# abignoli/EdgeGraph3D

Hardware: AMD Instinct MI355X
Metric: triangulated edge-points/sec (higher is better)
Workload: dtype f64

## Files before the change

edgegraph3d_amd/api.py:

```python
import ctypes as C
import os

import numpy as np

from . import _cdefs as D

_LIB = None


class Eg3dError(RuntimeError):
    pass


def lib_path():
    return os.environ.get("EG3D_LIB") or os.path.join(os.path.dirname(os.path.abspath(__file__)), "libeg3d.so")


def lib():
    global _LIB
    if _LIB is None:
        path = lib_path()
        if not os.path.exists(path):
            raise Eg3dError("libeg3d.so (HIP extension) is missing: run `python -m edgegraph3d_amd.build`. "
                            "There is no CPU fallback.")
        L = C.CDLL(path)
        L.eg3d_last_error.restype = C.c_char_p
        L.eg3d_device_count.restype = C.c_int
        L.eg3d_dlt_rows.restype = C.c_int
        L.eg3d_create.argtypes = [C.POINTER(D.Scene), C.c_int, C.POINTER(C.c_void_p)]
        L.eg3d_destroy.argtypes = [C.c_void_p]
        L.eg3d_clone.argtypes = [C.c_void_p, C.POINTER(C.c_void_p)]
        L.eg3d_get_grid.argtypes = [C.c_void_p, C.c_int, C.c_int, D.u32p, D.u32p, C.POINTER(D.u32p), C.POINTER(D.u32p)]
        L.eg3d_candidates_run.argtypes = [C.c_void_p, C.POINTER(D.Seeds), C.c_uint32, C.c_uint32, C.POINTER(D.Candidates)]
        L.eg3d_free_candidates.argtypes = [C.POINTER(D.Candidates)]
        L.eg3d_match_refpoints.argtypes = [C.c_void_p, C.POINTER(D.Seeds), C.c_uint32, C.c_uint32, C.c_int,
                                           C.POINTER(D.EdgePoints), C.POINTER(D.StageTimes)]
        L.eg3d_free_edgepoints.argtypes = [C.POINTER(D.EdgePoints)]
        L.eg3d_upload_seeds.argtypes = [C.c_void_p, C.POINTER(D.Seeds)]
        L.eg3d_match_resident.argtypes = [C.c_void_p, C.c_uint32, C.c_uint32, C.c_int, C.POINTER(D.EdgePoints),
                                          C.POINTER(D.StageTimes)]
        L.eg3d_match_polyline_sets.argtypes = [C.c_void_p, C.POINTER(D.PolylineSets), C.c_uint32, C.c_uint32, C.c_int,
                                               C.POINTER(D.EdgePoints), C.POINTER(D.StageTimes)]
        L.eg3d_check_polyline_sets.argtypes = [C.POINTER(D.PolylineSets), C.c_int32]
        L.eg3d_last_device_output.argtypes = [C.c_void_p, C.POINTER(D.DeviceEdgePoints)]
        L.eg3d_set_pipelining.argtypes = [C.c_void_p, C.c_int, C.c_int]
        L.eg3d_gn_filter.argtypes = [C.c_void_p, D.f32p, D.u32p, D.i32p, D.f32p, C.c_uint64, C.c_float, C.c_int,
                                     D.f32p, D.u8p, D.f32p]
        _LIB = L
    return _LIB


EXPORTED_SYMBOLS = [
    "eg3d_last_error", "eg3d_device_count", "eg3d_dlt_rows", "eg3d_create", "eg3d_clone", "eg3d_destroy", "eg3d_get_grid", "eg3d_candidates_run",
    "eg3d_free_candidates", "eg3d_match_refpoints", "eg3d_free_edgepoints", "eg3d_upload_seeds",
    "eg3d_match_resident", "eg3d_gn_filter", "eg3d_last_device_output", "eg3d_match_polyline_sets", "eg3d_check_polyline_sets", "eg3d_set_pipelining",
]


def _check(rc, what):
    if rc != 0:
        raise Eg3dError("%s failed (rc=%d): %s" % (what, rc, lib().eg3d_last_error().decode()))


def check_polyline_sets(n_sets, row_off, pl_ids, n_views):
    row_off = np.ascontiguousarray(row_off, np.uint32)
    pl_ids = np.ascontiguousarray(pl_ids if len(pl_ids) else [0], np.uint32)
    ps = D.PolylineSets(n_sets, D.np_ptr(row_off, C.c_uint32), D.np_ptr(pl_ids, C.c_uint32))
    _check(lib().eg3d_check_polyline_sets(C.byref(ps), n_views), "eg3d_check_polyline_sets")


def device_count():
    return int(lib().eg3d_device_count())


class Context:
    def __init__(self, scene_ptr, device=0, _handle=None):
        self._h = C.c_void_p()
        if _handle is not None:
            self._h = _handle
        else:
            _check(lib().eg3d_create(scene_ptr, device, C.byref(self._h)), "eg3d_create")

    def clone(self):
        h = C.c_void_p()
        _check(lib().eg3d_clone(self._h, C.byref(h)), "eg3d_clone")
        return Context(None, _handle=h)

    def set_pipelining(self, lanes=0, units=0):
        _check(lib().eg3d_set_pipelining(self._h, lanes, units), "eg3d_set_pipelining")

    def close(self):
        if self._h:
            lib().eg3d_destroy(self._h)
            self._h = C.c_void_p()

    def __del__(self):
        try:
            self.close()
        except Exception:
            pass

    def grid(self, view, which):
        ncols, nrows = C.c_uint32(), C.c_uint32()
        off, ids = D.u32p(), D.u32p()
        _check(lib().eg3d_get_grid(self._h, view, which, C.byref(ncols), C.byref(nrows), C.byref(off), C.byref(ids)),
               "eg3d_get_grid")
        n = ncols.value * nrows.value
        o = D.as_np(off, n + 1, np.uint32)
        return ncols.value, nrows.value, o, D.as_np(ids, int(o[-1]), np.uint32)

    def upload_seeds(self, seeds_ptr):
        _check(lib().eg3d_upload_seeds(self._h, seeds_ptr), "eg3d_upload_seeds")

    def match_resident(self, begin, end, device_only=False):
        e, tm = D.EdgePoints(), D.StageTimes()
        rc = lib().eg3d_match_resident(self._h, begin, end, 1 if device_only else 0, C.byref(e), C.byref(tm))
        _check(rc, "eg3d_match_resident")
        if device_only:
            d = {"n_points": int(e.n_points), "n_obs": int(e.n_obs), "n_tasks": int(e.n_tasks),
                 "n_hypotheses": int(e.n_hypotheses), "n_chains": int(e.n_chains), "flags": int(e.flags)}
        else:
            d = D.edgepoints_to_dict(e)
        lib().eg3d_free_edgepoints(C.byref(e))
        d["times"] = {f[0]: getattr(tm, f[0]) for f in D.StageTimes._fields_}
        return d

    def time_match_to_host(self, begin, end):
        import time
        e, tm = D.EdgePoints(), D.StageTimes()
        t0 = time.perf_counter()
        rc = lib().eg3d_match_resident(self._h, begin, end, 0, C.byref(e), C.byref(tm))
        dt = time.perf_counter() - t0
        _check(rc, "eg3d_match_resident")
        n = int(e.n_points)
        lib().eg3d_free_edgepoints(C.byref(e))
        return dt, n

    def time_match_sets_to_host(self, n_sets, row_off, pl_ids):
        import time
        row_off = np.ascontiguousarray(row_off, np.uint32)
        pl_ids = np.ascontiguousarray(pl_ids if len(pl_ids) else [0], np.uint32)
        ps = D.PolylineSets(n_sets, D.np_ptr(row_off, C.c_uint32), D.np_ptr(pl_ids, C.c_uint32))
# ... 109 lines not shown
```

edgegraph3d_amd/csrc/eg3d_api.hip:

```cpp
#include <hip/hip_runtime.h>
#include <hipcub/hipcub.hpp>

#include <algorithm>
#include <cstdio>
#include <cstdlib>
#include <sys/mman.h>

#include <atomic>
#include <chrono>
#include <cmath>
#include <condition_variable>
#include <cstring>
#include <memory>
#include <mutex>
#include <shared_mutex>
#include <string>
#include <thread>
#include <vector>

#include "../../include/eg3d.h"
#include "../../include/eg3d_host.h"
#include "eg3d_host_copy.h"
#include "eg3d_kernels.h"

// ... 25 lines not shown
      g_err = std::string("hipMalloc(") + std::to_string(want) + "): " + hipGetErrorString(e);
      return EG3D_ERR_HIP;
    }
    cap = want;
    return EG3D_OK;
  }
  int ensure_keep(size_t bytes, size_t keep, hipStream_t st) {
    if (bytes <= cap && p) return EG3D_OK;
    if (!p || !keep) return ensure(bytes);
    void* q = nullptr;
    const size_t want = bytes + bytes / 2;
    hipError_t e = hipMalloc(&q, want);
    if (e != hipSuccess) {
      g_err = std::string("hipMalloc(") + std::to_string(want) + "): " + hipGetErrorString(e);
      return EG3D_ERR_HIP;
    }
    e = hipMemcpyAsync(q, p, keep, hipMemcpyDeviceToDevice, st);
    if (e == hipSuccess) e = hipStreamSynchronize(st);
    if (e != hipSuccess) {
      (void)hipFree(q);
      g_err = std::string("growing a device buffer: ") + hipGetErrorString(e);
      return EG3D_ERR_HIP;
    }
    (void)hipFree(p);
    p = q;
    cap = want;
    return EG3D_OK;
  }
  void release() {
    if (p) (void)hipFree(p);
    p = nullptr;
    cap = 0;
  }
  template <typename T>
  T* as() const {
    return reinterpret_cast<T*>(p);
  }
};

#define BUF_TRY(expr)          \
  do {                         \
    int _r = (expr);           \
    if (_r != EG3D_OK) return _r; \
  } while (0)

struct DevOwner {
  int device = 0;
  std::vector<void*> ptrs;
  ~DevOwner() {
    (void)hipSetDevice(device);
    for (void* p : ptrs)
      if (p) (void)hipFree(p);
  }
};
struct HostGrids {
  std::mutex mu;
  bool have[2] = {false, false};
  std::vector<std::vector<uint32_t>> h_off[2], h_ids[2];
  int device = 0, n_views = 0;
  const uint32_t* d_off[2] = {nullptr, nullptr};
  const uint32_t* d_ids[2] = {nullptr, nullptr};
  uint32_t cells_per_view[2] = {0, 0};
};

#ifndef EG3D_K3B_ENGINE_DEFAULT
#define EG3D_K3B_ENGINE_DEFAULT 0
#endif
struct Tunables {
  bool grid_on_host = false;
  int lanes = 0, units = 0, test_fail_unit = 0;
  int copy_threads = 0;
  double unit_ramp = 0.6;
  int lane_priorities = 1;
  static constexpr int kHostCallLanes = 3;
  int k3a_engine_waves = 0, k3a_engine_lanes = 0;
  int k3b_engine = EG3D_K3B_ENGINE_DEFAULT, k3c_waves = 0, k3c_lanes = 0;
  bool assume_short = false;
  bool trace_arena = false;
  bool k3b_full = false;
  uint32_t arena_cap0 = 0, hyp_cap = 0;
  uint32_t chain_cap0 = 0, pool_cap0 = 0;
  size_t max_scratch = 0;
  uint32_t slots_per_xcd = 0;
  bool use_lpt = true;
  static Tunables from_env() {
    Tunables t;
    if (const char* e = getenv("EG3D_K3A_ENGINE_WAVES")) t.k3a_engine_waves = atoi(e);
    if (const char* e = getenv("EG3D_K3A_ENGINE_LANES")) t.k3a_engine_lanes = atoi(e);
    if (const char* e = getenv("EG3D_K3B_ENGINE")) t.k3b_engine = atoi(e);
    if (const char* e = getenv("EG3D_K3C_WAVES")) t.k3c_waves = atoi(e);
    if (const char* e = getenv("EG3D_K3C_LANES")) t.k3c_lanes = atoi(e);
    if (const char* e = getenv("EG3D_K3B_ASSUME_SHORT")) t.assume_short = e[0] == '1';
    if (const char* e = getenv("EG3D_HYP_CAP")) t.hyp_cap = (uint32_t)std::max(1, atoi(e));
    if (const char* e = getenv("EG3D_ARENA_CAP0")) t.arena_cap0 = (uint32_t)std::max(16, atoi(e));
    if (const char* e = getenv("EG3D_CHAIN_CAP0")) t.chain_cap0 = (uint32_t)std::max(8, atoi(e));
    if (const char* e = getenv("EG3D_POOL_CAP0")) t.pool_cap0 = (uint32_t)std::max(64, atoi(e));
    if (const char* e = getenv("EG3D_MAX_SCRATCH_MB")) t.max_scratch = (size_t)std::max(1, atoi(e)) << 20;
    if (const char* e = getenv("EG3D_NO_LPT")) t.use_lpt = !(e[0] == '1');
    if (const char* e = getenv("EG3D_TRACE_ARENA")) t.trace_arena = e[0] == '1';
    if (const char* e = getenv("EG3D_K3B_FULL")) t.k3b_full = e[0] == '1';
    if (const char* e = getenv("EG3D_SLOTS_PER_XCD")) t.slots_per_xcd = (uint32_t)std::max(1, atoi(e));
    if (const char* e = getenv("EG3D_PIPELINE_LANES")) t.lanes = std::min(16, std::max(0, atoi(e)));
    if (const char* e = getenv("EG3D_TEST_FAIL_UNIT")) t.test_fail_unit = atoi(e);
    if (const char* e = getenv("EG3D_GRID_ON_HOST")) t.grid_on_host = e[0] == '1';
    if (const char* e = getenv("EG3D_COPY_THREADS_PER_LANE")) t.copy_threads = std::min(32, std::max(1, atoi(e)));
    if (const char* e = getenv("EG3D_LANE_PRIORITIES")) t.lane_priorities = atoi(e);
    if (const char* e = getenv("EG3D_UNIT_RAMP")) t.unit_ramp = std::min(16.0, std::max(1.0 / 16.0, atof(e)));
    if (const char* e = getenv("EG3D_PIPELINE_UNITS")) t.units = std::min(4096, std::max(0, atoi(e)));
    return t;
  }
};

struct eg3d_ctx {
  int device = 0;
  Tunables tune;
  hipStream_t stream = nullptr;
  int V = 0, W = 0, H = 0;
  DevScene ds;
  DevBuf b_camP, b_F, b_Fv, b_vpo, b_pvo, b_vtx, b_pls, b_ple, b_g30o, b_g30i, b_g4o, b_g4i, b_bbo, b_bb;
  std::shared_ptr<DevOwner> scene_owner;
  std::shared_ptr<HostGrids> hg;
  uint32_t gw[2] = {0, 0}, gh[2] = {0, 0};
  uint32_t grid_dropped = 0;
  uint32_t n_seeds = 0;
  std::shared_ptr<std::vector<uint32_t>> h_trk;
  DevBuf b_toff, b_tview, b_txy;
  std::shared_ptr<DevOwner> seeds_owner;
  DevBuf b_sv_seed, b_map_view, b_map_entry, b_map_n, b_raw_cnt, b_raw_off, b_cand_pl, b_start_hits, b_cand_cnt,
      b_start_cnt, b_task_off, b_task_seed, b_task_entry, b_task_hit, b_task_k, b_task_list_off, b_list_cnt, b_list_ptr,
      b_hits, b_tasks, b_nhyp, b_hyp_off, b_res, b_arena, b_ctr, b_cs_task, b_valid, b_chain_off, b_chains,
      b_cscratch, b_couts, b_cpts, b_cobs, b_cpoff, b_cooff, b_scan_tmp, b_scanchk, b_cost, b_cidx, b_cost2, b_order, b_redo[2];
  DevBuf o_X, o_off, o_view, o_pl, o_seg, o_xy, o_key;
  DevBuf f_X, f_off, f_view, f_xy, f_Xo, f_inl;
  DevBuf b_sets_off, b_sets_ids;
  DevBuf b_fscratch, b_queue, b_items;
  DevBuf b_pools, b_stage_pts, b_stage_obs, b_stage_used;
  uint32_t slots_per_xcd = 0;
  int k3c_per_cu = 0;
  bool k3b_long_latched = false;
  uint32_t max_pl_vtx = 0;
  uint64_t stage_cap_pts = 0, stage_cap_obs = 0;
  hipEvent_t ea[8], eb[8];
  hipEvent_t ecopy[7] = {nullptr, nullptr, nullptr, nullptr, nullptr, nullptr, nullptr};
  uint32_t chain_cap = 384, pool_cap = 0, hyp_cap = 160;
  uint32_t n_simd = 0;
  int wall_clock_khz = 0;
  double arena_per_hyp = 16.0;
  void* pinned = nullptr;
  size_t pinned_cap = 0, ring_chunk = 0;
  uint32_t* mbox = nullptr;
  uint32_t* mbox_dev = nullptr;
  uint32_t mbox_seq = 0;
  uint64_t last_np = 0, last_no = 0;
  int last_chunks = 0;
  bool last_accumulated = false;
  uint32_t last_nc = 0;
  uint32_t last_nhyp = 0;
  std::vector<eg3d_ctx*> lanes;
  bool is_lane = false;
  uint32_t host_calls = 0;
  uint64_t last_host_cloud_bytes = 0;
};

#ifndef EG3D_D2H_CHUNK
#define EG3D_D2H_CHUNK ((size_t)16 << 20)
#endif
#define EG3D_D2H_CHUNK_SMALL ((size_t)2 << 20)
#define EG3D_D2H_BIG_CLOUD ((size_t)96 << 20)
#ifndef EG3D_D2H_RING
#define EG3D_D2H_RING 4
#endif
static int ensure_d2h_ring(eg3d_ctx* c, size_t cloud_bytes) {
  const size_t want = cloud_bytes >= EG3D_D2H_BIG_CLOUD ? EG3D_D2H_CHUNK : EG3D_D2H_CHUNK_SMALL;
  if (c->pinned && c->ring_chunk >= want) return EG3D_OK;
  if (c->pinned) (void)hipHostFree(c->pinned);
  c->pinned = nullptr;
  c->ring_chunk = c->pinned_cap = 0;
  HIP_TRY(hipHostMalloc(&c->pinned, want * EG3D_D2H_RING, hipHostMallocDefault));
  c->ring_chunk = want;
  c->pinned_cap = want * EG3D_D2H_RING;
  return EG3D_OK;
}

template <typename T>
static int upload(DevBuf& b, const T* src, size_t n, hipStream_t st) {
  BUF_TRY(b.ensure(sizeof(T) * std::max<size_t>(n, 1)));
  if (n) HIP_TRY(hipMemcpyAsync(b.p, src, sizeof(T) * n, hipMemcpyHostToDevice, st));
  return EG3D_OK;
}

static int scan_exclusive_u32(eg3d_ctx* c, const uint32_t* in, uint32_t* out, size_t n_plus_one) {
  size_t tmp_bytes = 0;
  HIP_TRY(hipcub::DeviceScan::ExclusiveSum(nullptr, tmp_bytes, in, out, (int)n_plus_one, c->stream));
  BUF_TRY(c->b_scan_tmp.ensure(tmp_bytes));
  HIP_TRY(hipcub::DeviceScan::ExclusiveSum(c->b_scan_tmp.p, tmp_bytes, in, out, (int)n_plus_one, c->stream));
  return EG3D_OK;
}
static int ensure_mailbox(eg3d_ctx* c) {
  if (!c->mbox) {
    void* h = nullptr;
    HIP_TRY(hipHostMalloc(&h, sizeof(uint32_t) * EG3D_MBOX_WORDS, hipHostMallocMapped | hipHostMallocCoherent));
    memset(h, 0, sizeof(uint32_t) * EG3D_MBOX_WORDS);
    void* d = nullptr;
    if (hipHostGetDevicePointer(&d, h, 0) != hipSuccess) {
      (void)hipHostFree(h);
      g_err = "eg3d: hipHostGetDevicePointer failed for the read-back mailbox";
      return EG3D_ERR_HIP;
    }
    c->mbox = (uint32_t*)h;
    c->mbox_dev = (uint32_t*)d;
  }
  if (!c->b_scanchk.p) {
    BUF_TRY(c->b_scanchk.ensure(8 * sizeof(uint32_t)));
    HIP_TRY(hipMemsetAsync(c->b_scanchk.p, 0, 8 * sizeof(uint32_t), c->stream));
  }
// ... 405 lines not shown
        rc = EG3D_ERR_HIP;
      }
      if (rc != EG3D_OK) ok = false;
    }
    if (!ok) {
      if (rc == EG3D_OK) {
        g_err = "eg3d_create: grid construction failed";
        rc = EG3D_ERR_ARG;
      }
      eg3d_destroy(c);
      return rc;
    }
  }
  d.g30_w = (int)c->gw[0];
  d.g30_h = (int)c->gh[0];
  d.g4_w = (int)c->gw[1];
  d.g4_h = (int)c->gh[1];
  d.g30_off = c->b_g30o.as<uint32_t>();
  d.g30_ids = c->b_g30i.as<uint32_t>();
  d.g4_off = c->b_g4o.as<uint32_t>();
  d.g4_ids = c->b_g4i.as<uint32_t>();
  {
    bool mid = true;
    for (size_t v = 0; v < (size_t)V && mid; v++)
      for (int k = 0; k < 12 && mid; k++) {
        const float p = sc->cam_P[v * 16 + k];
        if (p != 0.0f) {
          const float a = p < 0 ? -p : p;
          mid = a >= 7.888609052210118e-31f && a <= 1.2676506002282294e+30f;
        }
      }
    d.cams_mid_range = mid ? 1 : 0;
  }
  c->max_pl_vtx = 0;
  for (uint32_t p = 0; p < NP; p++)
    if (sc->pl_valid[p]) c->max_pl_vtx = std::max(c->max_pl_vtx, sc->pl_vtx_off[p + 1] - sc->pl_vtx_off[p]);
  c->pool_cap = std::min<uint32_t>(131072, 768u * (uint32_t)std::min(V, 128));
  if (c->pool_cap < 6144) c->pool_cap = 6144;
  if (c->tune.pool_cap0) c->pool_cap = c->tune.pool_cap0;
  if (c->tune.chain_cap0) c->chain_cap = c->tune.chain_cap0;
  hipDeviceProp_t prop;
  HIP_TRY(hipGetDeviceProperties(&prop, device));
  c->n_simd = (uint32_t)prop.multiProcessorCount * 4;
  if (hipDeviceGetAttribute(&c->wall_clock_khz, hipDeviceAttributeWallClockRate, device) != hipSuccess) c->wall_clock_khz = 0;
  {
    const int per_cu = k3b_blocks_per_cu();
    if (per_cu < 1) {
      g_err = "eg3d_create: occupancy query of the expand kernel failed";
      eg3d_destroy(c);
      return EG3D_ERR_HIP;
    }
    const uint32_t cus = (uint32_t)prop.multiProcessorCount;
    const uint32_t n_xcd = std::min(8u, std::max(1u, cus / 32u));
    const uint32_t cus_per_xcd = std::max<uint32_t>((cus + n_xcd - 1u) / n_xcd, 40u);
    c->slots_per_xcd = ((uint32_t)per_cu + 1u) * cus_per_xcd + 16u;
    if (c->tune.slots_per_xcd) c->slots_per_xcd = c->tune.slots_per_xcd;
    if (c->tune.k3b_engine != 0) {
#ifdef EG3D_WITH_K3C_ENGINE
      c->k3c_per_cu = k3c_blocks_per_cu();
      if (c->k3c_per_cu < 1) {
        g_err = "eg3d_create: occupancy query of the expand engine failed";
        eg3d_destroy(c);
        return EG3D_ERR_HIP;
      }
#else
      g_err = "eg3d_create: EG3D_K3B_ENGINE=1, but this library was built without the lane-per-chain engine "
              "(-DEG3D_WITH_K3C_ENGINE: edgegraph3d_amd/variants/libeg3d_engine.so)";
      eg3d_destroy(c);
      return EG3D_ERR_ARG;
#endif
    }
  }
  HIP_TRY(hipStreamSynchronize(c->stream));
  c->scene_owner = std::make_shared<DevOwner>();
  c->scene_owner->device = device;
  for (DevBuf* b : scene_bufs(c)) c->scene_owner->ptrs.push_back(b->p);
  *out = c;
  return EG3D_OK;
}

extern "C" int eg3d_clone(eg3d_ctx* parent, eg3d_ctx** out) {
  if (!parent || !out) {
    g_err = "eg3d_clone: bad arguments";
    return EG3D_ERR_ARG;
  }
  HIP_TRY(hipSetDevice(parent->device));
  eg3d_ctx* c = new eg3d_ctx();
  c->device = parent->device;
  c->tune = parent->tune;
  HIP_TRY(hipStreamCreateWithFlags(&c->stream, hipStreamNonBlocking));
  for (int i = 0; i < 8; i++) {
    HIP_TRY(hipEventCreate(&c->ea[i]));
    HIP_TRY(hipEventCreate(&c->eb[i]));
  }
  for (int i = 0; i < 7; i++) HIP_TRY(hipEventCreateWithFlags(&c->ecopy[i], hipEventDisableTiming));
  c->V = parent->V;
  c->W = parent->W;
  c->H = parent->H;
  c->ds = parent->ds;
  {
    std::vector<DevBuf*> src = scene_bufs(parent), dst = scene_bufs(c);
    for (size_t i = 0; i < src.size(); i++) *dst[i] = *src[i];
  }
  c->scene_owner = parent->scene_owner;
  c->hg = parent->hg;
  for (int k = 0; k < 2; k++) {
    c->gw[k] = parent->gw[k];
    c->gh[k] = parent->gh[k];
  }
  c->grid_dropped = parent->grid_dropped;
  c->n_seeds = parent->n_seeds;
  c->h_trk = parent->h_trk;
  c->b_toff = parent->b_toff;
  c->b_tview = parent->b_tview;
  c->b_txy = parent->b_txy;
  c->seeds_owner = parent->seeds_owner;
  c->chain_cap = parent->chain_cap;
  c->pool_cap = parent->pool_cap;
  c->hyp_cap = parent->hyp_cap;
  c->n_simd = parent->n_simd;
  c->wall_clock_khz = parent->wall_clock_khz;
  c->arena_per_hyp = parent->arena_per_hyp;
  c->slots_per_xcd = parent->slots_per_xcd;
  c->k3c_per_cu = parent->k3c_per_cu;
  c->k3b_long_latched = parent->k3b_long_latched;
  c->max_pl_vtx = parent->max_pl_vtx;
  c->stage_cap_pts = parent->stage_cap_pts;
  c->stage_cap_obs = parent->stage_cap_obs;
  *out = c;
  return EG3D_OK;
}

extern "C" void eg3d_destroy(eg3d_ctx* c) {
  if (!c) return;
  for (size_t l = 1; l < c->lanes.size(); l++) eg3d_destroy(c->lanes[l]);
  c->lanes.clear();
  (void)hipSetDevice(c->device);
  if (c->stream) (void)hipStreamSynchronize(c->stream);
  if (!c->scene_owner)
    for (DevBuf* b : scene_bufs(c)) b->release();
  c->scene_owner.reset();
  c->seeds_owner.reset();
  DevBuf* all[] = {&c->b_sv_seed, &c->b_map_view,
                   &c->b_map_entry, &c->b_map_n, &c->b_raw_cnt, &c->b_raw_off, &c->b_cand_pl, &c->b_start_hits,
                   &c->b_cand_cnt, &c->b_start_cnt, &c->b_task_off, &c->b_task_seed, &c->b_task_entry, &c->b_task_hit,
                   &c->b_task_k, &c->b_task_list_off, &c->b_list_cnt, &c->b_list_ptr, &c->b_hits, &c->b_tasks,
                   &c->b_nhyp, &c->b_hyp_off, &c->b_res, &c->b_arena, &c->b_ctr, &c->b_cs_task,
                   &c->b_valid, &c->b_chain_off, &c->b_chains, &c->b_cscratch, &c->b_couts, &c->b_cpts, &c->b_cobs,
                   &c->b_cpoff, &c->b_cooff, &c->b_scan_tmp, &c->b_scanchk, &c->b_cost, &c->b_cidx, &c->b_cost2, &c->b_order, &c->b_redo[0], &c->b_redo[1], &c->o_X, &c->o_off, &c->o_view, &c->o_pl, &c->o_seg,
                   &c->o_xy, &c->o_key, &c->f_X, &c->f_off, &c->f_view, &c->f_xy, &c->f_Xo, &c->f_inl, &c->b_sets_off, &c->b_sets_ids, &c->b_fscratch, &c->b_queue, &c->b_items,
                   &c->b_pools, &c->b_stage_pts, &c->b_stage_obs, &c->b_stage_used};
  for (DevBuf* b : all) b->release();
  if (c->pinned) (void)hipHostFree(c->pinned);
  if (c->mbox) (void)hipHostFree(c->mbox);
  for (int i = 0; i < 8; i++) {
    if (c->ea[i]) (void)hipEventDestroy(c->ea[i]);
    if (c->eb[i]) (void)hipEventDestroy(c->eb[i]);
  }
  for (int i = 0; i < 7; i++)
    if (c->ecopy[i]) (void)hipEventDestroy(c->ecopy[i]);
  if (c->stream) (void)hipStreamDestroy(c->stream);
  delete c;
}

extern "C" int eg3d_get_grid(eg3d_ctx* c, int view, int which, uint32_t* ncols, uint32_t* nrows,
                             const uint32_t** cell_off, const uint32_t** ids) {
  if (!c || view < 0 || view >= c->V || which < 0 || which > 1) {
    g_err = "eg3d_get_grid: bad arguments";
    return EG3D_ERR_ARG;
  }
  HostGrids& hg = *c->hg;
  {
    std::lock_guard<std::mutex> lk(hg.mu);
    if (!hg.have[which]) {
      HIP_TRY(hipSetDevice(hg.device));
      const size_t cpv = hg.cells_per_view[which], V = (size_t)hg.n_views;
      std::vector<uint32_t> off(V * cpv + 1);
      HIP_TRY(hipMemcpy(off.data(), hg.d_off[which], sizeof(uint32_t) * off.size(), hipMemcpyDeviceToHost));
      std::vector<uint32_t> all(std::max<size_t>(off.back(), 1));
      if (off.back()) HIP_TRY(hipMemcpy(all.data(), hg.d_ids[which], sizeof(uint32_t) * off.back(), hipMemcpyDeviceToHost));
      hg.h_off[which].resize(V);
      hg.h_ids[which].resize(V);
      for (size_t v = 0; v < V; v++) {
        const uint32_t base = off[v * cpv];
        hg.h_off[which][v].resize(cpv + 1);
        for (size_t cc = 0; cc <= cpv; cc++) hg.h_off[which][v][cc] = off[v * cpv + cc] - base;
        hg.h_ids[which][v].assign(all.begin() + base, all.begin() + off[(v + 1) * cpv]);
      }
      hg.have[which] = true;
    }
  }
  *ncols = c->gw[which];
  *nrows = c->gh[which];
  *cell_off = hg.h_off[which][(size_t)view].data();
  *ids = hg.h_ids[which][(size_t)view].data();
  return EG3D_OK;
}

extern "C" int eg3d_upload_seeds(eg3d_ctx* c, const eg3d_seeds* s) {
  if (!c || !s) {
    g_err = "eg3d_upload_seeds: bad arguments";
    return EG3D_ERR_ARG;
  }
  HIP_TRY(hipSetDevice(c->device));
// ... 311 lines not shown
  if (c->tune.arena_cap0) arena_cap = c->tune.arena_cap0;
  Counters hc;
  BUF_TRY(c->b_cs_task.ensure(sizeof(ChainSeed) * (nt + 1)));
  BUF_TRY(c->b_valid.ensure(sizeof(uint32_t) * (nt + 1)));
  BUF_TRY(c->b_chain_off.ensure(sizeof(uint32_t) * (nt + 1)));
  for (int attempt = 0;; attempt++) {
    BUF_TRY(c->b_arena.ensure(sizeof(HPoint) * (size_t)arena_cap));
    HIP_TRY(hipMemsetAsync(c->b_ctr.p, 0, 2 * sizeof(uint32_t), st));
    HIP_TRY(hipEventRecord(c->ea[3], st));
    HIP_TRY(hipMemsetAsync(c->b_queue.p, 0, 4 * sizeof(uint32_t), st));
    launch_k3a_engine(st, eng_waves, eng_waves, eng_lanes, c->ds, B.a, c->b_tasks.as<TaskDesc>(), c->b_hyp_off.as<uint32_t>(),
                      B.n_hyp, c->b_res.as<HypResult>(), c->b_fscratch.as<HPoint>(), c->hyp_cap, c->b_arena.as<HPoint>(),
                      arena_cap, c->b_ctr.as<Counters>(), c->b_queue.as<uint32_t>(), c->b_items.as<uint32_t>());
    HIP_TRY(hipEventRecord(c->eb[3], st));
    HIP_TRY(hipMemsetAsync(c->b_valid.as<uint32_t>() + nt, 0, sizeof(uint32_t), st));
    HIP_TRY(hipEventRecord(c->ea[4], st));
    launch_k3s(st, nt, c->b_hyp_off.as<uint32_t>(), c->b_res.as<HypResult>(), c->b_cs_task.as<ChainSeed>(),
               c->b_valid.as<uint32_t>());
    BUF_TRY(scan_queue_u32(c, c->b_valid.as<uint32_t>(), c->b_chain_off.as<uint32_t>(), nt + 1, 0));
    Readback rb(c);
    const int ic = rb.add(c->b_ctr.p, sizeof(Counters) / 4);
    const int it = rb.add(c->b_chain_off.as<uint32_t>() + nt, 1);
    const int iw = rb.add(c->b_scanchk.as<uint32_t>(), 1);
    rb.clear_after(c->b_scanchk.as<uint32_t>());
    BUF_TRY(rb.run());
    memcpy(&hc, rb.item(ic), sizeof(Counters));
    if (c->tune.trace_arena)
      fprintf(stderr, "eg3d: hypothesis arena: %u hypotheses, %u points used of %u (%.2f per hypothesis)%s\n", B.n_hyp,
              hc.arena_used, arena_cap, B.n_hyp ? (double)hc.arena_used / B.n_hyp : 0.0,
              (hc.flags & CTR_ARENA_OVERFLOW) ? " OVERFLOW" : "");
    if (!(hc.flags & CTR_ARENA_OVERFLOW)) {
      if (*rb.item(iw)) return wrapped_error("chains");
      B.n_chains = *rb.item(it);
      break;
    }
    if (attempt >= 6) {
      g_err = "eg3d: hypothesis arena overflow";
      return EG3D_ERR_CAPACITY;
    }
    arena_cap = std::max<uint32_t>(arena_cap * 2, hc.arena_used + (hc.arena_used >> 2));
    if (B.n_hyp) c->arena_per_hyp = std::max(c->arena_per_hyp, 1.25 * (double)arena_cap / (double)B.n_hyp);
  }
  H.flags |= (hc.flags & 0xffu);
  BUF_TRY(c->b_chains.ensure(sizeof(ChainSeed) * (B.n_chains + 1)));
  launch_compact_chains(st, nt, c->b_cs_task.as<ChainSeed>(), c->b_valid.as<uint32_t>(), c->b_chain_off.as<uint32_t>(),
                        c->b_chains.as<ChainSeed>());
  HIP_TRY(hipEventRecord(c->eb[4], st));
  const size_t max_scratch = c->tune.max_scratch;
  float ms_expand = 0, ms_emit = 0;
  uint32_t chunk = 0;
  uint32_t redo_n = 0, redo_nc = 0;
  int redo_buf = 0;
  for (uint32_t c0 = 0; c0 < B.n_chains; c0 += chunk) {
    const ChainLayout L = chain_layout(c->chain_cap, c->pool_cap, (uint32_t)c->V);
    chunk = redo_n ? redo_nc
                   : (uint32_t)std::max<size_t>(1, max_scratch ? std::min<size_t>(B.n_chains - c0, max_scratch / L.total)
                                                               : (size_t)(B.n_chains - c0));
    const uint32_t nc = std::min(chunk, B.n_chains - c0);
    BUF_TRY(ensure_mailbox(c));
    uint32_t* const saved_bytes = c->b_scanchk.as<uint32_t>() + 4;
    if (!redo_n)
      HIP_TRY(hipMemcpyAsync(saved_bytes, &c->b_ctr.as<Counters>()->bytes, sizeof(unsigned long long),
                             hipMemcpyDeviceToDevice, st));
#ifdef EG3D_WITH_K3C_ENGINE
    const bool engine = c->tune.k3b_engine != 0;
#else
    const bool engine = false;
#endif
    uint32_t eng_waves = 0, eng_lanes = 64;
    SlotPools pools;
    pools.base = nullptr;
    pools.stride = pools.ring_n = pools.slots_per_xcd = 0;
#ifdef EG3D_WITH_K3C_ENGINE
    if (engine) {
      const uint32_t per_simd = (uint32_t)(c->tune.k3c_waves > 0 ? c->tune.k3c_waves : std::max(1, c->k3c_per_cu / 4));
      const uint32_t waves_max = c->n_simd * per_simd;
      eng_lanes = c->tune.k3c_lanes > 0 ? (uint32_t)std::min(64, c->tune.k3c_lanes) : 8u;
      eng_waves = std::max<uint32_t>(1, std::min<uint32_t>(waves_max, (nc + eng_lanes - 1) / eng_lanes));
      while (eng_waves > 64 && L.total * (size_t)eng_waves * eng_lanes > ((size_t)16 << 30)) eng_waves /= 2;
      BUF_TRY(c->b_cscratch.ensure(L.total * (size_t)eng_waves * eng_lanes));
      BUF_TRY(c->b_queue.ensure(4 * sizeof(uint32_t)));
      HIP_TRY(hipMemsetAsync(c->b_queue.p, 0, 4 * sizeof(uint32_t), st));
    } else
#endif
    {
      BUF_TRY(c->b_cscratch.ensure(L.total * 8 * (size_t)c->slots_per_xcd));
      pools.slots_per_xcd = c->slots_per_xcd;
      pools.ring_n = 1;
      while (pools.ring_n <= c->slots_per_xcd) pools.ring_n <<= 1;
      pools.stride = 32 + pools.ring_n;
      BUF_TRY(c->b_pools.ensure(sizeof(uint32_t) * 8 * (size_t)pools.stride));
      pools.base = c->b_pools.as<uint32_t>();
      launch_pool_init(st, pools);
    }
    if (!redo_n) {
      const uint64_t guess_pts = 96ull * nc;
      const uint64_t per_pt = (uint64_t)std::min(100, std::max(8, c->V / 2));
      const uint64_t want_pts = std::max<uint64_t>(c->stage_cap_pts, guess_pts);
      const uint64_t want_obs = std::max<uint64_t>(c->stage_cap_obs, std::min<uint64_t>(guess_pts * per_pt, (8ull << 30) / sizeof(Obs)));
      BUF_TRY(c->b_stage_pts.ensure(sizeof(StagePt) * (size_t)want_pts));
      BUF_TRY(c->b_stage_obs.ensure(sizeof(Obs) * (size_t)want_obs));
      BUF_TRY(c->b_stage_used.ensure(2 * sizeof(unsigned long long)));
      HIP_TRY(hipMemsetAsync(c->b_stage_used.p, 0, 2 * sizeof(unsigned long long), st));
    }
    StageBuf stage;
    stage.pts = c->b_stage_pts.as<StagePt>();
    stage.obs = c->b_stage_obs.as<Obs>();
    stage.cap_pts = c->b_stage_pts.cap / sizeof(StagePt);
    stage.cap_obs = c->b_stage_obs.cap / sizeof(Obs);
    stage.used = c->b_stage_used.as<unsigned long long>();
    BUF_TRY(c->b_couts.ensure(sizeof(ChainOut) * (nc + 1)));
    BUF_TRY(c->b_cpts.ensure(sizeof(uint32_t) * (nc + 1)));
    BUF_TRY(c->b_cobs.ensure(sizeof(uint32_t) * (nc + 1)));
    BUF_TRY(c->b_cpoff.ensure(sizeof(uint32_t) * (nc + 1)));
    BUF_TRY(c->b_cooff.ensure(sizeof(uint32_t) * (nc + 1)));
    HIP_TRY(hipMemsetAsync(c->b_cpts.as<uint32_t>() + nc, 0, sizeof(uint32_t), st));
    HIP_TRY(hipMemsetAsync(c->b_cobs.as<uint32_t>() + nc, 0, sizeof(uint32_t), st));
    HIP_TRY(hipMemsetAsync(c->b_ctr.p, 0, 2 * sizeof(uint32_t), st));
    BUF_TRY(c->b_cost.ensure(sizeof(uint32_t) * (nc + 1)));
    BUF_TRY(c->b_cidx.ensure(sizeof(uint32_t) * (nc + 1)));
    BUF_TRY(c->b_cost2.ensure(sizeof(uint32_t) * (nc + 1)));
    BUF_TRY(c->b_order.ensure(sizeof(uint32_t) * (nc + 1)));
    const bool use_lpt = c->tune.use_lpt;
    const uint32_t n_launch = redo_n ? redo_n : nc;
    const uint32_t* const launch_order = redo_n ? c->b_redo[redo_buf].as<uint32_t>() : c->b_order.as<uint32_t>();
    if (!redo_n) {
    launch_chain_cost(st, B.a, c->b_tasks.as<TaskDesc>(), c->b_chains.as<ChainSeed>() + c0, nc, c->b_cost.as<uint32_t>(),
                      c->b_cidx.as<uint32_t>());
    {
      size_t tmp_bytes = 0;
      HIP_TRY(hipcub::DeviceRadixSort::SortPairsDescending(nullptr, tmp_bytes, c->b_cost.as<uint32_t>(),
                                                           c->b_cost2.as<uint32_t>(), c->b_cidx.as<uint32_t>(),
                                                           c->b_order.as<uint32_t>(), (int)nc, 0, 32, st));
      BUF_TRY(c->b_scan_tmp.ensure(tmp_bytes));
      HIP_TRY(hipcub::DeviceRadixSort::SortPairsDescending(c->b_scan_tmp.p, tmp_bytes, c->b_cost.as<uint32_t>(),
                                                           c->b_cost2.as<uint32_t>(), c->b_cidx.as<uint32_t>(),
                                                           c->b_order.as<uint32_t>(), (int)nc, 0, 32, st));
    }
    if (!use_lpt)
      HIP_TRY(hipMemcpyAsync(c->b_order.p, c->b_cidx.p, sizeof(uint32_t) * nc, hipMemcpyDeviceToDevice, st));
    }
    HIP_TRY(hipEventRecord(c->ea[5], st));
    const bool general = c->tune.k3b_full || c->k3b_long_latched || c->max_pl_vtx > EG3D_STAGE_VTX_HOST;
#ifdef EG3D_WITH_K3C_ENGINE
    if (engine)
      launch_k3c(st, eng_waves, eng_lanes, c->ds, B.a, c->b_tasks.as<TaskDesc>(), c->b_chains.as<ChainSeed>() + c0, nc,
                 c->b_hyp_off.as<uint32_t>(), c->b_res.as<HypResult>(), c->b_arena.as<HPoint>(), c->b_map_view.as<int32_t>(),
                 c->b_map_entry.as<uint32_t>(), c->b_map_n.as<uint32_t>(), L, c->b_cscratch.as<unsigned char>(), stage,
                 c->b_couts.as<ChainOut>(), c->b_cpts.as<uint32_t>(), c->b_cobs.as<uint32_t>(), c->b_ctr.as<Counters>(),
                 c->b_order.as<uint32_t>(), c->b_queue.as<uint32_t>(),
                 (c->tune.k3b_full || c->k3b_long_latched || (c->V > EG3D_SMALL_SCENE_VIEWS_HOST && !c->tune.assume_short)) ? 1 : 0);
    else
#endif
    launch_k3b(st, c->ds, B.a, c->b_tasks.as<TaskDesc>(), c->b_chains.as<ChainSeed>() + c0, n_launch,
               c->b_hyp_off.as<uint32_t>(), c->b_res.as<HypResult>(), c->b_arena.as<HPoint>(),
               c->b_map_view.as<int32_t>(), c->b_map_entry.as<uint32_t>(), c->b_map_n.as<uint32_t>(), L,
               c->b_cscratch.as<unsigned char>(), pools, stage, c->b_couts.as<ChainOut>(), c->b_cpts.as<uint32_t>(),
               c->b_cobs.as<uint32_t>(), c->b_ctr.as<Counters>(), launch_order,
               general ? 1 : (c->V > EG3D_SMALL_SCENE_VIEWS_HOST && !c->tune.assume_short) ? 2 : 0);
    HIP_TRY(hipEventRecord(c->eb[5], st));
    if (!device_only)
      BUF_TRY(ensure_d2h_ring(c, (size_t)nc * 50u * (36u + 20u * (size_t)std::min(c->V, 12))));
    BUF_TRY(scan_queue_u32(c, c->b_cpts.as<uint32_t>(), c->b_cpoff.as<uint32_t>(), nc + 1, 0));
    BUF_TRY(scan_queue_u32(c, c->b_cobs.as<uint32_t>(), c->b_cooff.as<uint32_t>(), nc + 1, 1));
    uint32_t np = 0, no = 0;
    unsigned long long stage_used[2] = {0, 0};
    {
      Readback rb(c);
      const int ic = rb.add(c->b_ctr.p, sizeof(Counters) / 4);
      const int ip = rb.add(c->b_cpoff.as<uint32_t>() + nc, 1);
      const int io = rb.add(c->b_cooff.as<uint32_t>() + nc, 1);
      const int iw = rb.add(c->b_scanchk.as<uint32_t>(), 2);
      const int iu = rb.add(c->b_stage_used.p, 4);
      rb.clear_after(c->b_scanchk.as<uint32_t>());
      rb.clear_after(c->b_scanchk.as<uint32_t>() + 1);
      BUF_TRY(rb.run());
      memcpy(&hc, rb.item(ic), sizeof(Counters));
      np = *rb.item(ip);
      no = *rb.item(io);
      memcpy(stage_used, rb.item(iu), sizeof(stage_used));
      const bool overflow = hc.flags & (EG3D_FLAG_CHAIN_OVERFLOW | EG3D_FLAG_OBS_OVERFLOW);
      if (!overflow && rb.item(iw)[0]) return wrapped_error("edge-points of one chunk");
      if (!overflow && rb.item(iw)[1]) return wrapped_error("observations of one chunk");
    }
    if (hc.flags & CTR_LONG_REFUSED) {
      if (c->k3b_long_latched) {
        g_err = "eg3d: internal: the general build of the expand kernel refused a solve";
        return EG3D_ERR_HIP;
      }
      c->k3b_long_latched = true;
      if (c->tune.trace_arena) fprintf(stderr, "eg3d: expand launch of %u chains redone: a solve of more than 32 rows -> general build\n", nc);
      HIP_TRY(hipMemcpyAsync(&c->b_ctr.as<Counters>()->bytes, saved_bytes, sizeof(unsigned long long),
                             hipMemcpyDeviceToDevice, st));
      HIP_TRY(hipStreamSynchronize(st));
      chunk = 0;
      redo_n = 0;
      continue;
    }
    if (hc.flags & CTR_SLOT_STARVED) {
      g_err = "eg3d: internal: the expand kernel found no free working slice (slot pool smaller than the residency)";
      return EG3D_ERR_HIP;
    }
    if (!(hc.flags & (EG3D_FLAG_CHAIN_OVERFLOW | EG3D_FLAG_OBS_OVERFLOW)) &&
        (np > stage.cap_pts || no > stage.cap_obs || stage_used[0] > stage.cap_pts || stage_used[1] > stage.cap_obs)) {
      if (c->tune.trace_arena)
        fprintf(stderr, "eg3d: expand launch of %u chains redone: staging area %zu points / %zu observations, needed %u / %u\n", nc,
                (size_t)stage.cap_pts, (size_t)stage.cap_obs, np, no);
      c->stage_cap_pts = std::max<uint64_t>(c->stage_cap_pts, std::max<uint64_t>(np, stage_used[0]) + np / 16 + 64);
      c->stage_cap_obs = std::max<uint64_t>(c->stage_cap_obs, std::max<uint64_t>(no, stage_used[1]) + no / 16 + 64);
      HIP_TRY(hipMemcpyAsync(&c->b_ctr.as<Counters>()->bytes, saved_bytes, sizeof(unsigned long long),
                             hipMemcpyDeviceToDevice, st));
      HIP_TRY(hipStreamSynchronize(st));
      chunk = 0;
      redo_n = 0;
      continue;
    }
    if (hc.flags & (EG3D_FLAG_CHAIN_OVERFLOW | EG3D_FLAG_OBS_OVERFLOW)) {
      const bool can_grow = ((hc.flags & EG3D_FLAG_CHAIN_OVERFLOW) && c->chain_cap < 8192) ||
                            ((hc.flags & EG3D_FLAG_OBS_OVERFLOW) && c->pool_cap < (1u << 20));
      if (can_grow) {
        if (hc.flags & EG3D_FLAG_CHAIN_OVERFLOW) c->chain_cap *= 2;
        if (hc.flags & EG3D_FLAG_OBS_OVERFLOW) c->pool_cap *= 2;
        H.flags |= hc.flags & 0xffu & ~(uint32_t)(EG3D_FLAG_CHAIN_OVERFLOW | EG3D_FLAG_OBS_OVERFLOW);
        {
          float t_launch = 0;
          HIP_TRY(hipEventElapsedTime(&t_launch, c->ea[5], c->eb[5]));
          ms_expand += t_launch;
        }
        uint32_t n_again = 0;
        if (!engine) {
          const int nb = redo_n ? 1 - redo_buf : 0;
          BUF_TRY(c->b_redo[nb].ensure(sizeof(uint32_t) * (nc + 1)));
          BUF_TRY(c->b_queue.ensure(4 * sizeof(uint32_t)));
          HIP_TRY(hipMemsetAsync(c->b_queue.p, 0, 4 * sizeof(uint32_t), st));
          launch_collect_overflow(st, c->b_couts.as<ChainOut>(), launch_order, n_launch, c->b_redo[nb].as<uint32_t>(),
                                  c->b_queue.as<uint32_t>(), c->b_ctr.as<Counters>());
          Readback rb(c);
          const int in = rb.add(c->b_queue.p, 1);
          BUF_TRY(rb.run());
          n_again = *rb.item(in);
          redo_buf = nb;
        }
        if (c->tune.trace_arena)
          fprintf(stderr, "eg3d: expand launch of %u chains: %u outgrew their slices (flags %u); relaunching %s with %u points / %u "
                          "observation slots per chain\n", n_launch, n_again, hc.flags & 3u, n_again ? "those" : "the chunk", c->chain_cap, c->pool_cap);
        if (n_again) {
          redo_n = n_again;
          redo_nc = nc;
        } else {
          redo_n = 0;
          HIP_TRY(hipMemcpyAsync(&c->b_ctr.as<Counters>()->bytes, saved_bytes, sizeof(unsigned long long),
                                 hipMemcpyDeviceToDevice, st));
// ... 399 lines not shown
  c->last_accumulated = device_only != 0;
  if (!device_only) {
    c->host_calls++;
    c->last_host_cloud_bytes = 36 * S.n_points + 20 * S.n_obs;
  }
  if (device_only) {
    c->last_np = S.n_points;
    c->last_no = S.n_obs;
  }
  if (!device_only) {
    const size_t npts = (size_t)S.n_points;
    if (!S.off.reserve(npts + 1)) {
      g_err = "eg3d: out of host memory for the edge-point cloud";
      return EG3D_ERR_ARG;
    }
    S.off[npts] = S.n_obs;
    out->X = S.X.release();
    out->obs_off = S.off.release();
    out->obs_view = S.view.release();
    out->obs_pl = S.pl.release();
    out->obs_seg = S.seg.release();
    out->obs_xy = S.xy.release();
    out->key = S.key.release();
    out->_owner = (void*)1;
  }
  if (times) {
    times->ms_total = total;
    times->ms_candidates = H.ms[1];
    times->ms_epipolar = H.ms[2];
    times->ms_hypotheses = H.ms[3];
    times->ms_select = H.ms[4];
    times->ms_expand = H.ms[5];
    times->ms_emit = H.ms[6];
    times->bytes_algorithmic = H.bytes_algorithmic + 12 * S.n_points + 20 * S.n_obs;
    times->ms_slowest_chain = c->wall_clock_khz > 0 ? (float)((double)H.max_chain_ticks / (double)c->wall_clock_khz) : 0.0f;
  }
  if (H.flags & (EG3D_FLAG_CHAIN_OVERFLOW | EG3D_FLAG_OBS_OVERFLOW | EG3D_FLAG_HYP_OVERFLOW)) {
    g_err = "eg3d: a device-side capacity was exceeded (flags in out->flags)";
    const uint32_t flags = out->flags;
    eg3d_free_edgepoints(out);
    out->flags = flags;
    return EG3D_ERR_CAPACITY;
  }
  return EG3D_OK;
}

extern "C" int eg3d_set_pipelining(eg3d_ctx* c, int lanes, int units) {
  if (!c || lanes < 0 || units < 0) {
    g_err = "eg3d_set_pipelining: bad arguments";
    return EG3D_ERR_ARG;
  }
  c->tune.lanes = std::min(16, lanes);
  c->tune.units = std::min(4096, units);
  return EG3D_OK;
}

static int lanes_for(const eg3d_ctx* c, int device_only) {
  if (c->tune.lanes > 0) return c->tune.lanes;
  if (device_only) return 1;
  const size_t arena = chain_layout(c->chain_cap, c->pool_cap, (uint32_t)c->V).total * 8 * (size_t)c->slots_per_xcd;
  if (arena > ((size_t)4 << 30)) return 1;
  return c->host_calls > 0 && c->last_host_cloud_bytes >= ((uint64_t)4 << 20) ? Tunables::kHostCallLanes : 1;
}

static std::vector<UnitRange> plan_seed_units(const eg3d_ctx* c, uint32_t b, uint32_t e, int lanes) {
  const uint32_t SEED_BATCH = 16384, MIN_UNIT = 128;
  const uint32_t n = e - b;
  const std::vector<uint32_t>& trk = *c->h_trk;
  auto cum = [&](uint32_t i) { return (double)trk[i] + 1e-3 * (double)i; };
  if (lanes <= 1 && !c->tune.units) {
    std::vector<UnitRange> out;
    for (uint32_t s0 = b; s0 < e; s0 += SEED_BATCH) {
      const uint32_t s1 = std::min(e, s0 + SEED_BATCH);
      out.push_back({s0, s1, cum(s1) - cum(s0)});
    }
    return out;
  }
  uint32_t n_units = c->tune.units ? (uint32_t)c->tune.units : std::min<uint32_t>((uint32_t)lanes, n / MIN_UNIT);
  n_units = std::max(n_units, (n + SEED_BATCH - 1) / SEED_BATCH);
  std::vector<UnitRange> out = cut_by_weight(b, e, std::max(1u, n_units), cum, c->tune.unit_ramp);
  for (size_t i = 0; i < out.size();) {
    if (out[i].e - out[i].b > SEED_BATCH) {
      const uint32_t mid = out[i].b + (out[i].e - out[i].b) / 2, end = out[i].e;
      out[i] = {out[i].b, mid, cum(mid) - cum(out[i].b)};
      out.insert(out.begin() + (long)i + 1, {mid, end, cum(end) - cum(mid)});
    } else {
      i++;
    }
  }
  return out;
}

extern "C" int eg3d_match_resident(eg3d_ctx* c, uint32_t b, uint32_t e, int device_only, eg3d_edgepoints* out,
                                   eg3d_stage_times* times) {
  if (!c || !out || b > e || e > c->n_seeds) {
    g_err = "eg3d_match_resident: bad arguments (seeds uploaded?)";
    return EG3D_ERR_ARG;
  }
  HIP_TRY(hipSetDevice(c->device));
  memset(out, 0, sizeof(*out));
  CallSink S;
  S.owner = c;
  S.device_only = device_only;
  c->last_np = c->last_no = 0;
  c->last_chunks = 0;
  const int lanes = lanes_for(c, device_only);
// ... 378 lines not shown
```

include/eg3d.h:

```cpp
#ifndef EG3D_H_
#define EG3D_H_

#include <stdint.h>
#include <stddef.h>

#ifdef __cplusplus
extern "C" {
#endif

#define EG3D_OK 0
#define EG3D_ERR_ARG -1
#define EG3D_ERR_HIP -2
#define EG3D_ERR_CAPACITY -3
#define EG3D_ERR_NODEVICE -4

typedef struct eg3d_scene {
  int32_t n_views;
  int32_t width, height;
  const float* cam_P;
  const double* F;
  const uint8_t* F_valid;
  const uint32_t* view_pl_off;
  const uint32_t* pl_vtx_off;
  const float* vtx_xy;
// ... 51 lines not shown
  void* _owner;
} eg3d_candidates;

typedef struct eg3d_ctx eg3d_ctx;

typedef struct eg3d_stage_times {
  float ms_total;
  float ms_candidates;
  float ms_epipolar;
  float ms_hypotheses;
  float ms_select;
  float ms_expand;
  float ms_emit;
  uint64_t bytes_algorithmic;
  float ms_slowest_chain;
} eg3d_stage_times;

const char* eg3d_last_error(void);
int eg3d_device_count(void);
int eg3d_dlt_rows(void);

int eg3d_create(const eg3d_scene* scene, int device, eg3d_ctx** out);
void eg3d_destroy(eg3d_ctx* ctx);

int eg3d_clone(eg3d_ctx* parent, eg3d_ctx** out);

int eg3d_get_grid(eg3d_ctx* ctx, int view, int which, uint32_t* ncols, uint32_t* nrows,
                  const uint32_t** cell_off, const uint32_t** ids);

int eg3d_candidates_run(eg3d_ctx* ctx, const eg3d_seeds* seeds, uint32_t seed_begin,
                        uint32_t seed_end, eg3d_candidates* out);
void eg3d_free_candidates(eg3d_candidates* c);

int eg3d_match_refpoints(eg3d_ctx* ctx, const eg3d_seeds* seeds, uint32_t seed_begin,
                         uint32_t seed_end, int device_only, eg3d_edgepoints* out,
                         eg3d_stage_times* times );
typedef struct eg3d_polyline_sets {
  uint32_t n_sets;
  const uint32_t* row_off;
  const uint32_t* pl_ids;
} eg3d_polyline_sets;
int eg3d_match_polyline_sets(eg3d_ctx* ctx, const eg3d_polyline_sets* sets, uint32_t set_begin, uint32_t set_end,
                             int device_only, eg3d_edgepoints* out, eg3d_stage_times* times);
int eg3d_check_polyline_sets(const eg3d_polyline_sets* sets, int32_t n_views);

void eg3d_free_edgepoints(eg3d_edgepoints* e);

int eg3d_upload_seeds(eg3d_ctx* ctx, const eg3d_seeds* seeds);
int eg3d_match_resident(eg3d_ctx* ctx, uint32_t seed_begin, uint32_t seed_end, int device_only,
                        eg3d_edgepoints* out, eg3d_stage_times* times);

int eg3d_set_pipelining(eg3d_ctx* ctx, int lanes, int units);

typedef struct eg3d_device_edgepoints {
  uint64_t n_points, n_obs;
  const float* X;
  const uint64_t* obs_off;
  const int32_t* obs_view;
  const uint32_t* obs_pl;
  const uint32_t* obs_seg;
  const float* obs_xy;
  const uint32_t* key;
  int32_t complete;
} eg3d_device_edgepoints;
int eg3d_last_device_output(eg3d_ctx* ctx, eg3d_device_edgepoints* out);

int eg3d_gn_filter(eg3d_ctx* ctx, const float* X, const uint32_t* obs_off, const int32_t* obs_view,
                   const float* obs_xy, uint64_t n_points, float gn_max_mse, int legacy_abs,
                   float* X_out, uint8_t* inlier, float* ms_kernel );

#ifdef __cplusplus
}
#endif
#endif
```

Before: 46.45 million.

## Share a persistent expand-stage slot arena across cloned contexts and drop per-chunk pool init

Moves the expand kernel's per-slot scratch slices and slot pools into a shared arena owned by a context family, so cloned contexts reuse one allocation and the pool is initialised once instead of on every chunk. It also changes the slots-per-XCD sizing formula, removing the +1 per-CU slack and the 40-CU floor on full XCDs, which shrinks the arena. Together these cut per-chunk launch and memset overhead and the memory footprint. In exchange, contexts share one pool under a mutex, and the tighter slot count risks slot starvation, which now retires the arena before returning an error.

```diff
diff --git a/edgegraph3d_amd/api.py b/edgegraph3d_amd/api.py
--- a/edgegraph3d_amd/api.py
+++ b/edgegraph3d_amd/api.py
@@ -44,6 +44,8 @@
         L.eg3d_check_polyline_sets.argtypes = [C.POINTER(D.PolylineSets), C.c_int32]
         L.eg3d_last_device_output.argtypes = [C.c_void_p, C.POINTER(D.DeviceEdgePoints)]
         L.eg3d_set_pipelining.argtypes = [C.c_void_p, C.c_int, C.c_int]
+        L.eg3d_arena_info.argtypes = [C.c_void_p, C.POINTER(C.c_uint64), C.POINTER(C.c_uint64), C.POINTER(C.c_uint32),
+                                      C.POINTER(C.c_int)]
         L.eg3d_gn_filter.argtypes = [C.c_void_p, D.f32p, D.u32p, D.i32p, D.f32p, C.c_uint64, C.c_float, C.c_int,
                                      D.f32p, D.u8p, D.f32p]
         _LIB = L
@@ -54,6 +56,7 @@
     "eg3d_last_error", "eg3d_device_count", "eg3d_dlt_rows", "eg3d_create", "eg3d_clone", "eg3d_destroy", "eg3d_get_grid", "eg3d_candidates_run",
     "eg3d_free_candidates", "eg3d_match_refpoints", "eg3d_free_edgepoints", "eg3d_upload_seeds",
     "eg3d_match_resident", "eg3d_gn_filter", "eg3d_last_device_output", "eg3d_match_polyline_sets", "eg3d_check_polyline_sets", "eg3d_set_pipelining",
+    "eg3d_arena_info",
 ]
 
 
@@ -88,6 +91,11 @@
 
     def set_pipelining(self, lanes=0, units=0):
         _check(lib().eg3d_set_pipelining(self._h, lanes, units), "eg3d_set_pipelining")
+
+    def arena_info(self):
+        a, s, n, on = C.c_uint64(), C.c_uint64(), C.c_uint32(), C.c_int()
+        _check(lib().eg3d_arena_info(self._h, C.byref(a), C.byref(s), C.byref(n), C.byref(on)), "eg3d_arena_info")
+        return {"arena_bytes": a.value, "slice_bytes": s.value, "slots_per_xcd": n.value, "allocated": bool(on.value)}
 
     def close(self):
         if self._h:
diff --git a/edgegraph3d_amd/csrc/eg3d_api.hip b/edgegraph3d_amd/csrc/eg3d_api.hip
--- a/edgegraph3d_amd/csrc/eg3d_api.hip
+++ b/edgegraph3d_amd/csrc/eg3d_api.hip
@@ -101,6 +101,23 @@
     for (void* p : ptrs)
       if (p) (void)hipFree(p);
   }
+};
+struct SliceArena {
+  int device = 0;
+  uint32_t chain_cap = 0, pool_cap = 0;
+  size_t bytes = 0;
+  unsigned char* slices = nullptr;
+  SlotPools pools{nullptr, 0, 0, 0};
+  ~SliceArena() {
+    (void)hipSetDevice(device);
+    if (slices) (void)hipFree(slices);
+    if (pools.base) (void)hipFree(pools.base);
+  }
+};
+struct ArenaFamily {
+  std::mutex mu;
+  std::shared_ptr<SliceArena> cur;
+  uint32_t chain_cap = 0, pool_cap = 0;
 };
 struct HostGrids {
   std::mutex mu;
@@ -183,7 +200,9 @@
   DevBuf f_X, f_off, f_view, f_xy, f_Xo, f_inl;
   DevBuf b_sets_off, b_sets_ids;
   DevBuf b_fscratch, b_queue, b_items;
-  DevBuf b_pools, b_stage_pts, b_stage_obs, b_stage_used;
+  std::shared_ptr<ArenaFamily> arena_family;
+  std::shared_ptr<SliceArena> slice_arena;
+  DevBuf b_stage_pts, b_stage_obs, b_stage_used;
   uint32_t slots_per_xcd = 0;
   int k3c_per_cu = 0;
   bool k3b_long_latched = false;
@@ -210,6 +229,43 @@
   uint32_t host_calls = 0;
   uint64_t last_host_cloud_bytes = 0;
 };
+
+static int adopt_slice_arena(eg3d_ctx* c, hipStream_t st) {
+  ArenaFamily& f = *c->arena_family;
+  std::lock_guard<std::mutex> lk(f.mu);
+  c->chain_cap = f.chain_cap = std::max(c->chain_cap, f.chain_cap);
+  c->pool_cap = f.pool_cap = std::max(c->pool_cap, f.pool_cap);
+  if (f.cur && f.cur->chain_cap == c->chain_cap && f.cur->pool_cap == c->pool_cap) {
+    c->slice_arena = f.cur;
+    return EG3D_OK;
+  }
+  c->slice_arena.reset();
+  f.cur.reset();
+  auto a = std::make_shared<SliceArena>();
+  a->device = c->device;
+  a->chain_cap = c->chain_cap;
+  a->pool_cap = c->pool_cap;
+  a->pools.slots_per_xcd = c->slots_per_xcd;
+  a->pools.ring_n = 1;
+  while (a->pools.ring_n <= c->slots_per_xcd) a->pools.ring_n <<= 1;
+  a->pools.stride = 32 + a->pools.ring_n;
+  a->bytes = chain_layout(c->chain_cap, c->pool_cap, (uint32_t)c->V).total * 8 * (size_t)c->slots_per_xcd;
+  hipError_t e = hipMalloc((void**)&a->slices, a->bytes);
+  if (e == hipSuccess) e = hipMalloc((void**)&a->pools.base, sizeof(uint32_t) * 8 * (size_t)a->pools.stride);
+  if (e != hipSuccess) {
+    g_err = std::string("hipMalloc of the expand stage's slot arena (") + std::to_string(a->bytes) + " bytes): " + hipGetErrorString(e);
+    return EG3D_ERR_HIP;
+  }
+  launch_pool_init(st, a->pools);
+  HIP_TRY(hipStreamSynchronize(st));
+  c->slice_arena = f.cur = a;
+  return EG3D_OK;
+}
+static void retire_slice_arena(eg3d_ctx* c) {
+  std::lock_guard<std::mutex> lk(c->arena_family->mu);
+  if (c->arena_family->cur == c->slice_arena) c->arena_family->cur.reset();
+  c->slice_arena.reset();
+}
 
 #ifndef EG3D_D2H_CHUNK
 #define EG3D_D2H_CHUNK ((size_t)16 << 20)
@@ -721,8 +777,9 @@
     }
     const uint32_t cus = (uint32_t)prop.multiProcessorCount;
     const uint32_t n_xcd = std::min(8u, std::max(1u, cus / 32u));
-    const uint32_t cus_per_xcd = std::max<uint32_t>((cus + n_xcd - 1u) / n_xcd, 40u);
-    c->slots_per_xcd = ((uint32_t)per_cu + 1u) * cus_per_xcd + 16u;
+    uint32_t cus_per_xcd = (cus + n_xcd - 1u) / n_xcd;
+    if (cus % 32u) cus_per_xcd = std::max(cus_per_xcd, 40u);
+    c->slots_per_xcd = (uint32_t)per_cu * cus_per_xcd + 16u;
     if (c->tune.slots_per_xcd) c->slots_per_xcd = c->tune.slots_per_xcd;
     if (c->tune.k3b_engine != 0) {
 #ifdef EG3D_WITH_K3C_ENGINE
@@ -741,6 +798,7 @@
     }
   }
   HIP_TRY(hipStreamSynchronize(c->stream));
+  c->arena_family = std::make_shared<ArenaFamily>();
   c->scene_owner = std::make_shared<DevOwner>();
   c->scene_owner->device = device;
   for (DevBuf* b : scene_bufs(c)) c->scene_owner->ptrs.push_back(b->p);
@@ -772,6 +830,7 @@
     for (size_t i = 0; i < src.size(); i++) *dst[i] = *src[i];
   }
   c->scene_owner = parent->scene_owner;
+  c->arena_family = parent->arena_family;
   c->hg = parent->hg;
   for (int k = 0; k < 2; k++) {
     c->gw[k] = parent->gw[k];
@@ -810,6 +869,8 @@
     for (DevBuf* b : scene_bufs(c)) b->release();
   c->scene_owner.reset();
   c->seeds_owner.reset();
+  c->slice_arena.reset();
+  c->arena_family.reset();
   DevBuf* all[] = {&c->b_sv_seed, &c->b_map_view,
                    &c->b_map_entry, &c->b_map_n, &c->b_raw_cnt, &c->b_raw_off, &c->b_cand_pl, &c->b_start_hits,
                    &c->b_cand_cnt, &c->b_start_cnt, &c->b_task_off, &c->b_task_seed, &c->b_task_entry, &c->b_task_hit,
@@ -818,7 +879,7 @@
                    &c->b_valid, &c->b_chain_off, &c->b_chains, &c->b_cscratch, &c->b_couts, &c->b_cpts, &c->b_cobs,
                    &c->b_cpoff, &c->b_cooff, &c->b_scan_tmp, &c->b_scanchk, &c->b_cost, &c->b_cidx, &c->b_cost2, &c->b_order, &c->b_redo[0], &c->b_redo[1], &c->o_X, &c->o_off, &c->o_view, &c->o_pl, &c->o_seg,
                    &c->o_xy, &c->o_key, &c->f_X, &c->f_off, &c->f_view, &c->f_xy, &c->f_Xo, &c->f_inl, &c->b_sets_off, &c->b_sets_ids, &c->b_fscratch, &c->b_queue, &c->b_items,
-                   &c->b_pools, &c->b_stage_pts, &c->b_stage_obs, &c->b_stage_used};
+                   &c->b_stage_pts, &c->b_stage_obs, &c->b_stage_used};
   for (DevBuf* b : all) b->release();
   if (c->pinned) (void)hipHostFree(c->pinned);
   if (c->mbox) (void)hipHostFree(c->mbox);
@@ -1236,6 +1297,12 @@
   uint32_t redo_n = 0, redo_nc = 0;
   int redo_buf = 0;
   for (uint32_t c0 = 0; c0 < B.n_chains; c0 += chunk) {
+#ifdef EG3D_WITH_K3C_ENGINE
+    const bool engine = c->tune.k3b_engine != 0;
+#else
+    const bool engine = false;
+#endif
+    if (!engine) BUF_TRY(adopt_slice_arena(c, st));
     const ChainLayout L = chain_layout(c->chain_cap, c->pool_cap, (uint32_t)c->V);
     chunk = redo_n ? redo_nc
                    : (uint32_t)std::max<size_t>(1, max_scratch ? std::min<size_t>(B.n_chains - c0, max_scratch / L.total)
@@ -1246,15 +1313,7 @@
     if (!redo_n)
       HIP_TRY(hipMemcpyAsync(saved_bytes, &c->b_ctr.as<Counters>()->bytes, sizeof(unsigned long long),
                              hipMemcpyDeviceToDevice, st));
-#ifdef EG3D_WITH_K3C_ENGINE
-    const bool engine = c->tune.k3b_engine != 0;
-#else
-    const bool engine = false;
-#endif
     uint32_t eng_waves = 0, eng_lanes = 64;
-    SlotPools pools;
-    pools.base = nullptr;
-    pools.stride = pools.ring_n = pools.slots_per_xcd = 0;
 #ifdef EG3D_WITH_K3C_ENGINE
     if (engine) {
       const uint32_t per_simd = (uint32_t)(c->tune.k3c_waves > 0 ? c->tune.k3c_waves : std::max(1, c->k3c_per_cu / 4));
@@ -1265,18 +1324,8 @@
       BUF_TRY(c->b_cscratch.ensure(L.total * (size_t)eng_waves * eng_lanes));
       BUF_TRY(c->b_queue.ensure(4 * sizeof(uint32_t)));
       HIP_TRY(hipMemsetAsync(c->b_queue.p, 0, 4 * sizeof(uint32_t), st));
-    } else
+    }
 #endif
-    {
-      BUF_TRY(c->b_cscratch.ensure(L.total * 8 * (size_t)c->slots_per_xcd));
-      pools.slots_per_xcd = c->slots_per_xcd;
-      pools.ring_n = 1;
-      while (pools.ring_n <= c->slots_per_xcd) pools.ring_n <<= 1;
-      pools.stride = 32 + pools.ring_n;
-      BUF_TRY(c->b_pools.ensure(sizeof(uint32_t) * 8 * (size_t)pools.stride));
-      pools.base = c->b_pools.as<uint32_t>();
-      launch_pool_init(st, pools);
-    }
     if (!redo_n) {
       const uint64_t guess_pts = 96ull * nc;
       const uint64_t per_pt = (uint64_t)std::min(100, std::max(8, c->V / 2));
@@ -1339,7 +1388,7 @@
     launch_k3b(st, c->ds, B.a, c->b_tasks.as<TaskDesc>(), c->b_chains.as<ChainSeed>() + c0, n_launch,
                c->b_hyp_off.as<uint32_t>(), c->b_res.as<HypResult>(), c->b_arena.as<HPoint>(),
                c->b_map_view.as<int32_t>(), c->b_map_entry.as<uint32_t>(), c->b_map_n.as<uint32_t>(), L,
-               c->b_cscratch.as<unsigned char>(), pools, stage, c->b_couts.as<ChainOut>(), c->b_cpts.as<uint32_t>(),
+               c->slice_arena->slices, c->slice_arena->pools, stage, c->b_couts.as<ChainOut>(), c->b_cpts.as<uint32_t>(),
                c->b_cobs.as<uint32_t>(), c->b_ctr.as<Counters>(), launch_order,
                general ? 1 : (c->V > EG3D_SMALL_SCENE_VIEWS_HOST && !c->tune.assume_short) ? 2 : 0);
     HIP_TRY(hipEventRecord(c->eb[5], st));
@@ -1382,6 +1431,7 @@
       continue;
     }
     if (hc.flags & CTR_SLOT_STARVED) {
+      retire_slice_arena(c);
       g_err = "eg3d: internal: the expand kernel found no free working slice (slot pool smaller than the residency)";
       return EG3D_ERR_HIP;
     }
@@ -1887,6 +1937,21 @@
   }
   c->tune.lanes = std::min(16, lanes);
   c->tune.units = std::min(4096, units);
+  return EG3D_OK;
+}
+
+extern "C" int eg3d_arena_info(eg3d_ctx* c, uint64_t* arena_bytes, uint64_t* slice_bytes, uint32_t* slots_per_xcd, int* allocated) {
+  if (!c || !c->arena_family) {
+    g_err = "eg3d_arena_info: bad arguments";
+    return EG3D_ERR_ARG;
+  }
+  ArenaFamily& f = *c->arena_family;
+  std::lock_guard<std::mutex> lk(f.mu);
+  const size_t slice = chain_layout(std::max(c->chain_cap, f.chain_cap), std::max(c->pool_cap, f.pool_cap), (uint32_t)c->V).total;
+  if (arena_bytes) *arena_bytes = (uint64_t)slice * 8u * c->slots_per_xcd;
+  if (slice_bytes) *slice_bytes = (uint64_t)slice;
+  if (slots_per_xcd) *slots_per_xcd = c->slots_per_xcd;
+  if (allocated) *allocated = f.cur ? 1 : 0;
   return EG3D_OK;
 }
 
diff --git a/include/eg3d.h b/include/eg3d.h
--- a/include/eg3d.h
+++ b/include/eg3d.h
@@ -127,6 +127,8 @@
 
 int eg3d_set_pipelining(eg3d_ctx* ctx, int lanes, int units);
 
+int eg3d_arena_info(eg3d_ctx* ctx, uint64_t* arena_bytes, uint64_t* slice_bytes, uint32_t* slots_per_xcd, int* allocated);
+
 typedef struct eg3d_device_edgepoints {
   uint64_t n_points, n_obs;
   const float* X;
```

New measurement: 46.44 million. Within noise of the previous version (-0.0%).
